# AO33/HiC_Genome_Assembler

Hardware: AMD Instinct MI355X
Metric: Part1+Part2 wall-clock (s) and bins/s on N x N contact map (higher is better)
Workload: dtype f64

## Files before the change

hic_genome_assembler_amd/csrc/api.hip:

```cpp
#include <hip/hip_runtime.h>

#include <algorithm>
#include <cmath>
#include <cstdarg>
#include <climits>
#include <cstdio>
#include <cstdlib>
#include <cstring>
#include <numeric>
#include <string>
#include <unordered_map>
#include <functional>
#include <chrono>
#include <vector>

#include "../../include/hicmi.h"
#include "hicmi_internal.h"
#include "hyper.h"

using namespace hicmi;

static thread_local std::string g_err;

static int fail(int code, const char* fmt, ...)
// ... 1150 lines not shown
    const uint16_t* src = c->dRank + row0 * c->ldr;
    HIPCHK(hipMemcpy2DAsync(out, sizeof(uint16_t) * (size_t)c->n, src, sizeof(uint16_t) * (size_t)c->ldr,
                            sizeof(uint16_t) * (size_t)c->n, (size_t)nrows, hipMemcpyDeviceToHost, c->stream));
    HIPCHK(sync_stream(c));
    if (!inverse) {
        std::vector<uint16_t> tmp((size_t)c->n);
        for (int64_t r = 0; r < nrows; r++) {
            uint16_t* row = out + r * c->n;
            for (int64_t col = 0; col < c->n; col++) {
                if (row[col] >= c->n) return fail(HICMI_ESTATE, "rank row %lld is not a permutation (a row of another shard?)", (long long)(row0 + r));
                tmp[row[col]] = (uint16_t)col;
            }
            memcpy(row, tmp.data(), sizeof(uint16_t) * (size_t)c->n);
        }
    }
    return HICMI_OK;
}

int hicmi_get_similarity_row(hicmi_ctx* c, int64_t row, double* out)
{
    if (!c || !out) return fail(HICMI_EINVAL, "bad arguments");
    if (!c->have_rank) return fail(HICMI_EINVAL, "hicmi_rank_matrix has not run");
    if (row < 0 || row >= c->n) return fail(HICMI_EINVAL, "row out of range");
    HIPCHK(hipSetDevice(c->device));
    int rc = ensure(c->d_tmp, c->tmp_cap, c->n);
    if (rc) return rc;
    launch_similarity_row(c->dC, c->ldc, c->d_order, c->d_np, c->d_seq, (int)c->n, (int)row, c->d_tmp, c->stream);
    HIPCHK(hipGetLastError());
    HIPCHK(hipMemcpyAsync(out, c->d_tmp, sizeof(double) * (size_t)c->n, hipMemcpyDeviceToHost, c->stream));
    HIPCHK(sync_stream(c));
    return HICMI_OK;
}

static int ensure_scan_buffers(hicmi_ctx* c)
{
    if (c->x_cap >= c->n && c->d_x && c->d_sig) return HICMI_OK;
    free_dev(c->d_x); free_dev(c->d_sig); c->d_x = nullptr; c->d_sig = nullptr; c->x_cap = 0;
    HIPCHK(hipMalloc((void**)&c->d_x, sizeof(int32_t) * (size_t)c->n));
    HIPCHK(hipMalloc((void**)&c->d_sig, (size_t)c->n));
    c->x_cap = c->n;
    return HICMI_OK;
}

static int finish_scan(hicmi_ctx* c, int64_t rows, int mode, int64_t L_fixed, int64_t M, double psig, int32_t* x_out,
                       uint8_t* sig_out, int64_t own_first)
{
    const bool direct = sig_out && !x_out;
    if (direct) { int rc = ensure_pin_down(c, (size_t)rows); if (rc) return rc; }
    {
        Timed t(c, F_HYPER_FLAGS, 5.0 * (double)rows);
        launch_hyper_flags(c->d_x, (int)rows, mode, (int)L_fixed, M, psig, direct ? reinterpret_cast<uint8_t*>(c->pin_down) : c->d_sig,
                           (int)own_first, (int)c->shard_stride, c->stream);
    }
    HIPCHK(hipGetLastError());
    if (direct) {
        HIPCHK(sync_stream(c));
        memcpy(sig_out, c->pin_down, (size_t)rows);
        return HICMI_OK;
    }
    if (x_out) { int rc = download(c, x_out, c->d_x, sizeof(int32_t) * (size_t)rows); if (rc) return rc; }
    if (sig_out) { int rc = download(c, sig_out, c->d_sig, (size_t)rows); if (rc) return rc; }
    if (!x_out && !sig_out) HIPCHK(sync_stream(c));
    return HICMI_OK;
}

int hicmi_cut_scan(hicmi_ctx* c, int64_t start, int64_t M, double psig, int32_t* x_out, uint8_t* sig_out)
{
    if (!c) return fail(HICMI_EINVAL, "NULL context");
    if (!c->have_rank) return fail(HICMI_EINVAL, "hicmi_rank_matrix has not run");
    const int64_t n = c->n;
    if (start < 0 || start >= n) return fail(HICMI_EINVAL, "start out of range");
    HIPCHK(hipSetDevice(c->device));
    int rc = ensure_scan_buffers(c);
    if (rc) return rc;
    const int64_t cnt = n - start;
    const int64_t st = c->shard_stride;
    const int64_t t0 = ((c->shard_first - start) % st + st) % st;
    if (c->cached_start != start) {
        HIPCHK(hipMemsetAsync(c->d_x, 0, sizeof(int32_t) * (size_t)(st > 1 ? cnt : 1), c->stream));
        const double m = (double)(cnt - 1);
        Timed t(c, F_CUT_COUNT, 2.0 * (m * (m + 3.0) / 2.0) / (double)st);
        const int64_t t1 = t0 >= 1 ? t0 : t0 + st;
        if (t1 < cnt)
            launch_cut_count(c->dRank, c->ldr, (int)(start + t1), (int)(cnt - t1), (int)start, 0, 0, c->d_x + t1, (int)st, c->stream);
        HIPCHK(hipGetLastError());
        c->cached_start = start;
    }
    return finish_scan(c, cnt, 0, 0, M, psig, x_out, sig_out, t0);
}

int hicmi_filter_scan(hicmi_ctx* c, int64_t start, int64_t cut, int64_t n_rows, int64_t M, double psig,
                      int32_t* x_out, uint8_t* sig_out)
{
    if (!c) return fail(HICMI_EINVAL, "NULL context");
    if (!c->have_rank) return fail(HICMI_EINVAL, "hicmi_rank_matrix has not run");
    const int64_t n = c->n;
    if (start < 0 || start >= n || cut < start || cut >= n || n_rows < 0 || start + n_rows > n)
        return fail(HICMI_EINVAL, "filter scan arguments out of range");
    HIPCHK(hipSetDevice(c->device));
    int rc = ensure_scan_buffers(c);
    if (rc) return rc;
    c->cached_start = -1;
    const int64_t st = c->shard_stride;
    const int64_t t0 = ((c->shard_first - start) % st + st) % st;
    if (st > 1) HIPCHK(hipMemsetAsync(c->d_x, 0, sizeof(int32_t) * (size_t)n_rows, c->stream));
    {
        Timed t(c, F_CUT_COUNT, 2.0 * (double)n_rows * (double)(cut - start + 1) / (double)st);
        if (t0 < n_rows)
            launch_cut_count(c->dRank, c->ldr, (int)(start + t0), (int)(n_rows - t0), (int)start, 1, (int)cut, c->d_x + t0, (int)st,
                             c->stream);
    }
    HIPCHK(hipGetLastError());
    return finish_scan(c, n_rows, 1, cut - start, M, psig, x_out, sig_out, t0);
}

double hicmi_hypergeom_sf(int64_t x, int64_t M, int64_t n, int64_t N) { return hypergeom_sf_ge(x, M, n, N); }
int hicmi_hypergeom_decide(int64_t x, int64_t M, int64_t n, int64_t N, double psig) { return hypergeom_decide(x, M, n, N, psig); }

static_assert(SCAN_MAX_SETS == HICMI_SCAN_MAX_SETS, "hicmi.h and the kernels disagree on the set cap");

struct ScanMulti {
    ScanState* st; int32_t *x, *cuts, *mlog, *alt, *seg, *seg_x; uint8_t *sig, *filt, *prev;
};

static int ensure_scan_multi(hicmi_ctx* c, int sets, ScanMulti& m)
{
    const size_t n = (size_t)c->n, S = (size_t)sets;
    const size_t head = (sizeof(ScanState) * SCAN_MAX_SETS + 255) & ~(size_t)255;
    const size_t bytes = head + S * n * (sizeof(int32_t) * 9 + 3) + 64;
    if (c->scan_multi_bytes < bytes || !c->d_scan_multi) {
        free_dev(c->d_scan_multi); c->d_scan_multi = nullptr; c->scan_multi_bytes = 0;
        HIPCHK(hipMalloc((void**)&c->d_scan_multi, bytes));
        c->scan_multi_bytes = bytes;
    }
    unsigned char* b = c->d_scan_multi;
    m.st = reinterpret_cast<ScanState*>(b);
    m.x = reinterpret_cast<int32_t*>(b + head);
    m.cuts = m.x + S * n; m.mlog = m.cuts + S * n; m.alt = m.mlog + 2 * S * n; m.seg = m.alt + S * n; m.seg_x = m.seg + 3 * S * n;
    m.sig = reinterpret_cast<uint8_t*>(m.seg_x + S * n); m.filt = m.sig + S * n; m.prev = m.filt + S * n;
    return HICMI_OK;
}

static int scan_share()
{
    const char* e = getenv("HICMI_SCAN_SHARE");
    return e && !strcmp(e, "0") ? 0 : 1;
}

static int run_scan_multi(hicmi_ctx* c, std::vector<ScanState>& h, const ScanMulti& m, const std::vector<int64_t>& max_scans,
                          const std::function<void(int)>& enqueue)
{
    const size_t S = h.size();
    int rc = upload(c, m.st, h.data(), sizeof(ScanState) * S);
    if (rc) return rc;
    const int pairs = 32;
    int64_t batches = 0;
    for (int64_t issued = 0; ; issued += pairs) {
        bool all_done = true;
        for (size_t k = 0; k < S; k++) {
            if (h[k].done) continue;
            all_done = false;
            if (issued > max_scans[k] + pairs)
                return fail(HICMI_ESTATE, "scan loop of set %d did not end after %lld scans", (int)k, (long long)issued);
        }
        if (all_done) break;
        {
            Timed t(c, F_CUT_COUNT, 0.0);
            enqueue(pairs);
        }
        HIPCHK(hipGetLastError());
        batches++;
        rc = download(c, h.data(), m.st, sizeof(ScanState) * S);
        if (rc) return rc;
    }
    int64_t scans = 0; double bytes = 0;
    for (const ScanState& r : h) { scans += r.scans; bytes += (double)r.bytes; }
    c->launches[F_CUT_COUNT] += scans - batches;
    c->launches[F_HYPER_FLAGS] += scans;
    c->bytes[F_CUT_COUNT] += bytes;
    return HICMI_OK;
}

static ScanState first_pass_record(int64_t n, int64_t min_size, int64_t stop_ind, double psig)
{
    ScanState r;
    memset(&r, 0, sizeof(r));
    r.mode = 0; r.start = 0; r.M = n; r.recount = 1; r.psig = psig;
    r.min_size = (int)std::min<int64_t>(min_size, n + 1); r.stop_ind = (int)std::min<int64_t>(stop_ind, INT32_MAX);
    return r;
}

static ScanState filter_record(int64_t n, int64_t n_in, int32_t first, double psig)
{
    ScanState r;
    memset(&r, 0, sizeof(r));
    r.mode = 1; r.start = 0; r.M = n; r.recount = 1; r.psig = psig;
    r.MD = (int)(n / 5);
    r.n_alt = (int)n_in; r.f_max_rounds = (int)std::min<int64_t>(10 * n_in, INT32_MAX);
    r.cut = first;
    r.n_rows = (int)std::min<int64_t>(n, (int64_t)r.MD + 1);
    r.done = n_in == 0;
    return r;
}

int hicmi_first_pass_cuts(hicmi_ctx* c, int64_t min_size, int64_t stop_ind, double psig, int32_t* cuts_out, int64_t cuts_cap,
                          int64_t* n_cuts_out, int32_t* m_log_out, int64_t log_cap, int64_t* n_log_out)
{
    return hicmi_first_pass_cuts_multi(c, 1, &min_size, &stop_ind, psig, cuts_out, cuts_cap, n_cuts_out, m_log_out, log_cap,
                                       n_log_out);
}

int hicmi_filter_cuts(hicmi_ctx* c, const int32_t* cuts_in, int64_t n_in, double psig, int32_t* cuts_out, int64_t cuts_cap,
                      int64_t* n_out, int64_t* warned_out)
{
    if (!c || !cuts_in || !cuts_out || !n_out || n_in < 1) return fail(HICMI_EINVAL, "bad arguments");
    const int64_t cand_off[2] = {0, n_in};
    int64_t warned = 0;
    const int rc = hicmi_filter_cuts_multi(c, 1, cand_off, cuts_in, &psig, cuts_out, cuts_cap, n_out, &warned);
    if (!rc && warned_out) *warned_out = warned;
    return rc;
}

int hicmi_first_pass_cuts_multi(hicmi_ctx* c, int64_t n_sets, const int64_t* min_size, const int64_t* stop_ind, double psig,
                                int32_t* cuts_out, int64_t cuts_cap, int64_t* n_cuts_out, int32_t* m_log_out, int64_t log_cap,
                                int64_t* n_log_out)
{
    if (!c || !min_size || !stop_ind || !cuts_out || !n_cuts_out || !n_log_out || (log_cap > 0 && !m_log_out))
        return fail(HICMI_EINVAL, "bad arguments");
    if (n_sets < 1 || n_sets > SCAN_MAX_SETS) return fail(HICMI_EINVAL, "n_sets must be in [1, %d]", SCAN_MAX_SETS);
    if (!c->have_rank) return fail(HICMI_EINVAL, "hicmi_rank_matrix has not run");
    if (c->shard_stride != 1) return fail(HICMI_EINVAL, "the device-driven scan loops need the whole rank matrix (no row shard)");
    for (int64_t k = 0; k < n_sets; k++)
        if (min_size[k] < 1) return fail(HICMI_EINVAL, "min_size must be >= 1 (set %lld)", (long long)k);
    const int64_t n = c->n;
    HIPCHK(hipSetDevice(c->device));
    ScanMulti m;
    int rc = ensure_scan_multi(c, (int)n_sets, m);
    if (rc) return rc;
    std::vector<ScanState> h((size_t)n_sets);
    for (int64_t k = 0; k < n_sets; k++) h[(size_t)k] = first_pass_record(n, min_size[k], stop_ind[k], psig);
    const int lcap = (int)n;
    const int share = scan_share();
    rc = run_scan_multi(c, h, m, std::vector<int64_t>((size_t)n_sets, 6 * n), [&](int pairs) {
        launch_first_pass_multi_pairs(c->dRank, c->ldr, (int)n, (int)n_sets, m.st, m.x, m.sig, psig, share, m.cuts, m.mlog,
                                      lcap, pairs, c->stream);
    });
    if (rc) return rc;
    for (int64_t k = 0; k < n_sets; k++) {
        const ScanState& r = h[(size_t)k];
        if (r.n_cuts > cuts_cap) return fail(HICMI_EINVAL, "%d cuts of set %lld do not fit cuts_cap", r.n_cuts, (long long)k);
        if (r.n_log > lcap || r.n_log > log_cap) return fail(HICMI_EINVAL, "%d M changes of set %lld do not fit the log", r.n_log, (long long)k);
    }
    for (int64_t k = 0; k < n_sets; k++) {
        const ScanState& r = h[(size_t)k];
        if (r.n_cuts) { rc = download(c, cuts_out + k * cuts_cap, m.cuts + k * n, sizeof(int32_t) * (size_t)r.n_cuts); if (rc) return rc; }
        if (r.n_log) { rc = download(c, m_log_out + 2 * k * log_cap, m.mlog + 2 * k * n, sizeof(int32_t) * 2 * (size_t)r.n_log); if (rc) return rc; }
        n_cuts_out[k] = r.n_cuts; n_log_out[k] = r.n_log;
    }
    return HICMI_OK;
}

int hicmi_filter_cuts_multi(hicmi_ctx* c, int64_t n_sets, const int64_t* cand_off, const int32_t* cuts_in, const double* psig,
                            int32_t* cuts_out, int64_t cuts_cap, int64_t* n_out, int64_t* warned_out)
{
    if (!c || !cand_off || !psig || !cuts_out || !n_out || !warned_out) return fail(HICMI_EINVAL, "bad arguments");
    if (n_sets < 1 || n_sets > SCAN_MAX_SETS) return fail(HICMI_EINVAL, "n_sets must be in [1, %d]", SCAN_MAX_SETS);
    if (!c->have_rank) return fail(HICMI_EINVAL, "hicmi_rank_matrix has not run");
    if (c->shard_stride != 1) return fail(HICMI_EINVAL, "the device-driven scan loops need the whole rank matrix (no row shard)");
    const int64_t n = c->n;
    if (cand_off[0] != 0) return fail(HICMI_EINVAL, "cand_off[0] must be 0");
    for (int64_t k = 0; k < n_sets; k++) {
        const int64_t a = cand_off[k], b = cand_off[k + 1];
        if (b < a || b - a > n) return fail(HICMI_EINVAL, "candidate list %lld: bad offsets", (long long)k);
        if (b > a && !cuts_in) return fail(HICMI_EINVAL, "bad arguments");
        for (int64_t i = a; i < b; i++)
            if (cuts_in[i] < 0 || cuts_in[i] >= n || (i > a && cuts_in[i] <= cuts_in[i - 1]))
                return fail(HICMI_EINVAL, "cuts must be ascending indices in [0, n) (set %lld)", (long long)k);
    }
    HIPCHK(hipSetDevice(c->device));
    ScanMulti m;
    int rc = ensure_scan_multi(c, (int)n_sets, m);
    if (rc) return rc;
    HIPCHK(hipMemsetAsync(m.filt, 0, 2 * (size_t)n_sets * (size_t)n, c->stream));
    std::vector<ScanState> h((size_t)n_sets);
    std::vector<int64_t> max_scans((size_t)n_sets);
    const int max_rows = (int)std::min<int64_t>(n, n / 5 + 1);
    for (int64_t k = 0; k < n_sets; k++) {
        const int64_t a = cand_off[k], n_in = cand_off[k + 1] - a;
        h[(size_t)k] = filter_record(n, n_in, n_in ? cuts_in[a] : 0, psig[k]);
        max_scans[(size_t)k] = std::min<int64_t>((int64_t)4000000, 20 * n_in * n_in * 10 + 1000);
        if (n_in) { rc = upload(c, m.alt + k * n, cuts_in + a, sizeof(int32_t) * (size_t)n_in); if (rc) return rc; }
    }
    const int share = scan_share();
    rc = run_scan_multi(c, h, m, max_scans, [&](int pairs) {
        launch_filter_multi_pairs(c->dRank, c->ldr, (int)n, max_rows, (int)n_sets, m.st, m.x, m.sig, psig[0], share, m.alt,
                                  m.filt, m.prev, m.seg, m.seg_x, pairs, c->stream);
    });
    if (rc) return rc;
    std::vector<uint8_t> kept((size_t)n_sets * (size_t)n);
    rc = download(c, kept.data(), m.filt, kept.size());
    if (rc) return rc;
    for (int64_t k = 0; k < n_sets; k++) {
        int64_t cnt = 0;
        const uint8_t* f = kept.data() + (size_t)k * (size_t)n;
        for (int64_t e = 0; e < n; e++)
            if (f[e]) {
                if (cnt >= cuts_cap) return fail(HICMI_EINVAL, "filtered cuts of set %lld do not fit cuts_cap", (long long)k);
                cuts_out[k * cuts_cap + cnt++] = (int32_t)e;
            }
        n_out[k] = cnt;
        warned_out[k] = h[(size_t)k].f_warned;
    }
    return HICMI_OK;
}

namespace {
void harmonic_table(std::vector<double>& H, int64_t n)
{
    H.assign((size_t)(n + 1), 0.0);
    for (int64_t k = 1; k <= n; k++) H[(size_t)k] = H[(size_t)k - 1] + 1.0 / (double)k;
}

int select_enqueue(hicmi_ctx* c, const int32_t* sel, int64_t n, const std::vector<double>* H_shared)
{
    if (!c || !sel || n < 1) return fail(HICMI_EINVAL, "bad arguments");
    if (!c->dC) return fail(HICMI_EINVAL, "no contact matrix set");
    for (int64_t i = 0; i < n; i++)
        if (sel[i] < 0 || sel[i] >= c->n) return fail(HICMI_EINVAL, "selection index out of range");
    HIPCHK(hipSetDevice(c->device));
// ... 2143 lines not shown
```

hic_genome_assembler_amd/csrc/hicmi_internal.h:

```cpp
#pragma once
#include <hip/hip_runtime.h>
#include <stdint.h>

#include <atomic>
#include <functional>

namespace hicmi {

inline void ensure_dynamic_lds(const void* func, std::atomic<int>& have, size_t bytes)
{
    if ((int)bytes > have.load(std::memory_order_relaxed)) {
        (void)hipFuncSetAttribute(func, hipFuncAttributeMaxDynamicSharedMemorySize, (int)bytes);
        have.store((int)bytes, std::memory_order_relaxed);
    }
}

static constexpr int SERIAL_BATCH = 16;

__device__ __forceinline__ double serial_sum_lds(const double* t, int from, int to, double acc)
{
    constexpr int B = SERIAL_BATCH;
    int i = from;
    if (i + B <= to) {
        double a[B];
// ... 88 lines not shown
    int dcap = 256;
    bool dcap_forced = false;
    bool compact = true;
    bool wgs_set = false; int wgs = 0;
    bool plain = false;
    bool gsize = false;
    bool w1 = true;
    int w1_s = 0;
    int w1_cols = 0;
    int w1_maxs = 0;
    int xcc = -1;
    int test_late = 0, test_diverge = 0, test_rollcall = 0;
};
NNChainOptions nnchain_options(int probed_xcc);
int nnchain_probe_xcc(hipStream_t s);
int launch_nnchain(double* W, double* W2, int64_t ldw, int n, int* chain, double* zraw, void* workspace, const NNChainOptions& o,
                   int fallback, hipStream_t s, const std::function<void()>& after_first_rowmin = nullptr);
void launch_selftest_division(unsigned long long seed, int blocks, int iters, unsigned long long* d_mismatches, hipStream_t s);
const int* nnchain_state_ptr(void* workspace);
const unsigned long long* nnchain_prof_ptr(void* workspace);
void launch_cut_count(const uint16_t* rank, int64_t ldr, int row0, int nrows, int lo, int mode, int cparam,
                      int32_t* x_out, int row_step, hipStream_t s);
void launch_hyper_flags(const int32_t* x, int nrows, int mode, int L_fixed, int64_t M, double psig, uint8_t* sig,
                        int own_first, int own_step, hipStream_t s);

struct ScanState {
    int done;
    int mode;
    int start, cut, n_rows, recount;
    long long M;
    double psig;
    int min_size, stop_ind, loop_count, n_cuts, n_log, scans;
    int MD, n_alt, alt_off, f_i, f_keep_from, f_noise, f_round, f_max_rounds, f_warned;
    int pad;
    unsigned long long bytes;
};
static constexpr int SCAN_MAX_SETS = 64;
void launch_first_pass_multi_pairs(const uint16_t* rank, int64_t ldr, int n, int n_sets, ScanState* st, int32_t* x, uint8_t* sig,
                                   double psig0, int share, int32_t* cuts, int32_t* mlog, int log_cap, int pairs, hipStream_t s);
void launch_filter_multi_pairs(const uint16_t* rank, int64_t ldr, int n, int max_rows, int n_sets, ScanState* st, int32_t* x,
                               uint8_t* sig, double psig0, int share, int32_t* alt, uint8_t* filt, uint8_t* prev,
                               int32_t* seg, int32_t* seg_x, int pairs, hipStream_t s);

#if defined(__HIPCC__)
template <int M>
__device__ __forceinline__ uint32_t xor_lane(uint32_t v, int lane)
{
    if constexpr (M == 1) return (uint32_t)__builtin_amdgcn_mov_dpp((int)v, 0xB1, 0xf, 0xf, true);
    else if constexpr (M == 2) return (uint32_t)__builtin_amdgcn_mov_dpp((int)v, 0x4E, 0xf, 0xf, true);
    else if constexpr (M == 4) {
        const int t = __builtin_amdgcn_mov_dpp((int)v, 0x141, 0xf, 0xf, true);
        return (uint32_t)__builtin_amdgcn_mov_dpp(t, 0x1B, 0xf, 0xf, true);
    } else if constexpr (M == 8) {
        const int t = __builtin_amdgcn_mov_dpp((int)v, 0x140, 0xf, 0xf, true);
        return (uint32_t)__builtin_amdgcn_mov_dpp(t, 0x141, 0xf, 0xf, true);
    } else if constexpr (M == 16) {
        const auto r = __builtin_amdgcn_permlane16_swap(v, v, false, false);
        return (lane & 16) ? r[0] : r[1];
    } else {
        static_assert(M == 32, "xor_lane: M must be 1, 2, 4, 8, 16 or 32");
        const auto r = __builtin_amdgcn_permlane32_swap(v, v, false, false);
        return (lane & 32) ? r[0] : r[1];
    }
}
#endif

int  sort_padded_size(int n);
int  sort_workgroups(int n);
size_t sort_scratch_bytes(int n);
struct SortExtras {
    const int32_t* row_list = nullptr; int n_list = 0;
    uint8_t* tie_flag = nullptr; unsigned* tie_count = nullptr; unsigned tie_limit = 0;
    uint16_t* tie_bits = nullptr; int64_t ld_bits = 0;
    int max_workgroups = 0;
    int avoid_xcc = -1; unsigned* row_counter = nullptr;
// ... 240 lines not shown
```

hic_genome_assembler_amd/csrc/k_part1_scan.hip:

```cpp
#include "hicmi_internal.h"
#include "hyper.h"

namespace hicmi {

__device__ __forceinline__ int row_count_partial(const uint16_t* __restrict__ r, int lo, int end, int thr, int tid)
{
    int cnt = 0;
    int body0 = (lo + 7) & ~7;
    if (body0 > end) body0 = end;
    const int body1 = body0 + ((end - body0) & ~7);
    for (int j = lo + tid; j < body0; j += 256) cnt += (int)r[j] < thr;
    for (int j = body0 + tid * 8; j < body1; j += 256 * 8) {
        uint4 q = *reinterpret_cast<const uint4*>(r + j);
        cnt += (int)(q.x & 0xffffu) < thr; cnt += (int)(q.x >> 16) < thr;
        cnt += (int)(q.y & 0xffffu) < thr; cnt += (int)(q.y >> 16) < thr;
        cnt += (int)(q.z & 0xffffu) < thr; cnt += (int)(q.z >> 16) < thr;
        cnt += (int)(q.w & 0xffffu) < thr; cnt += (int)(q.w >> 16) < thr;
    }
    for (int j = body1 + tid; j < end; j += 256) cnt += (int)r[j] < thr;
    return cnt;
}

__device__ __forceinline__ uint8_t row_flag(int mode, int total, long long M, int t, int thr, double psig)
{
// ... 2 lines not shown
}

__global__ __launch_bounds__(256) void k_cut_rows(const uint16_t* __restrict__ rank, int64_t ldr, int n,
                                                  const ScanState* __restrict__ st, int32_t* __restrict__ x,
                                                  uint8_t* __restrict__ sig, double psig)
{
    __shared__ int s_part[4];
    if (st->done) return;
    const int mode = st->mode, lo = st->start, t = blockIdx.x;
    const int rows = mode == 0 ? n - lo : st->n_rows;
    if (t >= rows) return;
    const int tid = threadIdx.x;
    if (mode == 0 && t == 0) { if (tid == 0) sig[0] = 0; return; }
    const int i = lo + t;
    const int hi = mode == 0 ? i : st->cut;
    const int thr = hi - lo;
    int total;
    if (st->recount) {
        int cnt = row_count_partial(rank + (int64_t)i * ldr, lo, hi + 1, thr, tid);
#pragma unroll
        for (int off = 32; off >= 1; off >>= 1) cnt += __shfl_xor(cnt, off, 64);
        if ((tid & 63) == 0) s_part[tid >> 6] = cnt;
        __syncthreads();
        if (tid != 0) return;
        total = s_part[0] + s_part[1] + s_part[2] + s_part[3];
        x[t] = total;
    } else {
        if (tid != 0) return;
        total = x[t];
    }
    sig[t] = row_flag(mode, total, st->M, t, thr, psig);
}

__device__ __forceinline__ void first_pass_decide(int n, ScanState* __restrict__ st, const uint8_t* __restrict__ sig,
                                                  int32_t* __restrict__ cuts, int32_t* __restrict__ mlog, int log_cap)
{
    __shared__ int s_sum[16];
    __shared__ int s_first;
    __shared__ int s_go;
    if (st->done) return;
    const int tid = threadIdx.x;
    const int start = st->start, cnt = n - start, h = st->min_size;
    int part = 0;
    for (int e = tid; e < cnt; e += 1024) part += sig[e];
#pragma unroll
    for (int off = 32; off >= 1; off >>= 1) part += __shfl_xor(part, off, 64);
    if ((tid & 63) == 0) s_sum[tid >> 6] = part;
    if (tid == 0) s_first = 0x7fffffff;
    __syncthreads();
    if (tid == 0) {
        int total = 0;
        for (int w = 0; w < 16; w++) total += s_sum[w];
        int go = 1;
        st->scans++;
        if (st->recount) { const unsigned long long m = (unsigned long long)(cnt - 1); st->bytes += m * (m + 3); }
        st->loop_count++;
        if ((double)total / (double)cnt >= .9) {
            const int64_t morg = st->M;
            st->M = morg - start;
            if (st->n_log < log_cap) { mlog[2 * st->n_log] = (int32_t)morg; mlog[2 * st->n_log + 1] = (int32_t)st->M; }
            st->n_log++;
            if (st->loop_count < 5) { go = 0; st->recount = 0; }
        }
        s_go = go;
    }
    __syncthreads();
    if (!s_go) return;
    const int full = cnt - 2 * h + 1;
    if (h < cnt) {
        for (int p = tid; p < full; p += 1024) {
            bool ok = true;
            for (int k = 0; k < h && ok; k++) ok = sig[p + k] == 1 && sig[p + h + k] == 0;
            if (ok) { atomicMin(&s_first, p); break; }
        }
    }
    __syncthreads();
    if (tid != 0) return;
    if (s_first == 0x7fffffff) { st->done = 1; return; }
    const int ind = start + s_first + h;
    cuts[st->n_cuts++] = ind;
    if (ind >= st->stop_ind || (n - ind) <= h) { st->done = 1; return; }
    st->start = ind; st->M = n - ind; st->loop_count = 0; st->recount = 1;
}

__device__ __forceinline__ void filter_begin_round(ScanState* st, int n)
{
    st->M = n - st->start;
    st->f_i = 0;
    st->f_keep_from = 0;
}

__device__ __forceinline__ void filter_set_scan(ScanState* st, const int32_t* alt, int n)
{
    st->cut = alt[st->alt_off + st->f_i];
    const int rest = n - st->start;
    st->n_rows = rest < st->MD + 1 ? rest : st->MD + 1;
    st->recount = 1;
}

static constexpr int FD_CAP = 2048;

__device__ __forceinline__ void filter_decide(int n, ScanState* __restrict__ st, const uint8_t* __restrict__ sig,
                                              int32_t* __restrict__ alt, uint8_t* __restrict__ filt,
                                              uint8_t* __restrict__ prev, int32_t* __restrict__ seg_g,
                                              int32_t* __restrict__ seg_x_g, double psig)
{
    __shared__ int s_alt[FD_CAP], s_seg[3 * FD_CAP], s_seg_x[FD_CAP];
    __shared__ int s_nseg, s_last, s_phase, s_diff, s_wave[16];
    if (st->done) return;
    const int tid = threadIdx.x;
    const int start = st->start, c = st->cut, n_rows = st->n_rows, n_alt = st->n_alt - st->alt_off;
    const bool in_lds = n_alt <= FD_CAP;
    int* a = in_lds ? s_alt : alt + st->alt_off;
    int* seg = in_lds ? s_seg : seg_g;
    int* seg_x = in_lds ? s_seg_x : seg_x_g;
    if (in_lds)
        for (int k = tid; k < n_alt; k += 1024) s_alt[k] = alt[st->alt_off + k];
    __syncthreads();
    if (tid == 0) {
        int ns = 0, fc_prev = start;
        for (int k = 0; k < n_alt; k++) {
            const int ai = a[k];
            if (ai == fc_prev) continue;
            const int lo = fc_prev, hi = ai;
            fc_prev = ai;
            if (hi <= lo) break;
            seg[3 * ns] = lo; seg[3 * ns + 1] = hi; seg[3 * ns + 2] = k;
            seg_x[ns] = 0;
            ns++;
        }
        s_nseg = ns; s_last = -1;
        st->scans++;
        st->bytes += 2ull * (unsigned long long)n_rows * (unsigned long long)(c - start + 1);
    }
    __syncthreads();
    const int ns = s_nseg;
    for (int e = tid; e < n_rows; e += 1024) {
        if (!sig[e]) continue;
        const int row = start + e;
        int lo_k = 0, hi_k = ns;
        while (lo_k < hi_k) {
            const int mid = (lo_k + hi_k) >> 1;
            if (seg[3 * mid + 1] > row) hi_k = mid; else lo_k = mid + 1;
        }
        if (lo_k < ns && seg[3 * lo_k] <= row) atomicAdd(&seg_x[lo_k], 1);
    }
    __syncthreads();
    const int64_t M = st->M;
    const int local = c - start;
    for (int k = tid; k < ns; k += 1024) {
        const double p = hypergeom_sf_ge((int64_t)seg_x[k], M, (int64_t)local, (int64_t)(seg[3 * k + 1] - seg[3 * k]));
        if (p < psig) atomicMax(&s_last, k);
    }
    __syncthreads();
    if (tid == 0) {
        int phase = 0;
        if (s_last >= 0) {
            st->f_keep_from = seg[3 * s_last + 2];
            st->start = seg[3 * s_last + 1];
            filt[st->start] = 1;
            st->f_noise = 1;
            phase = 1;
        } else {
            filt[c] = 1;
            st->f_keep_from = st->f_i;
            st->f_i++;
            if (st->f_i >= n_alt) phase = 1;
        }
        if (phase == 1) {
            st->f_round++;
            if (st->f_noise == 0) phase = 2;
            else {
                st->alt_off += st->f_keep_from;
                st->f_noise = 0;
                if (st->f_round >= st->f_max_rounds) { st->f_warned++; phase = 2; }
                else if (st->alt_off >= st->n_alt) phase = 2;
                else filter_begin_round(st, n);
            }
        }
        s_phase = phase;
        s_diff = 0;
    }
    __syncthreads();
    if (s_phase != 2) {
        if (tid == 0) filter_set_scan(st, alt, n);
        return;
    }
    __threadfence_block();
    const int chunk = (n + 1023) / 1024;
    const int e0 = tid * chunk, e1 = e0 + chunk < n ? e0 + chunk : n;
    int mine = 0, diff = 0;
    for (int e = e0; e < e1; e++) { const int f = filt[e]; mine += f; diff |= f != prev[e]; }
    if (diff) s_diff = 1;
    int incl = mine;
#pragma unroll
    for (int d = 1; d < 64; d <<= 1) { const int o = __shfl_up(incl, d, 64); if ((tid & 63) >= d) incl += o; }
    if ((tid & 63) == 63) s_wave[tid >> 6] = incl;
    __syncthreads();
    if (!s_diff) { if (tid == 0) st->done = 1; return; }
    int base = incl - mine, total = 0;
// ... 49 lines not shown
    }
    __syncthreads();
    const int items = s_pre[n_sets];
    for (int w = blockIdx.x; w < items; w += gridDim.x) {
        int k = 0;
        while (s_pre[k + 1] <= w) k++;
        const int t = w - s_pre[k];
        const int mode = s_key[k][1], lo = s_key[k][2];
        if (mode == 0 && t == 0) {
            if (tid < n_sets && s_lead[tid] == k) sig[(size_t)tid * n] = 0;
            continue;
        }
        const int i = lo + t;
        const int hi = mode == 0 ? i : st[k].cut;
        const int thr = hi - lo;
        if (s_key[k][3] >= 0) {
            int cnt = row_count_partial(rank + (int64_t)i * ldr, lo, hi + 1, thr, tid);
#pragma unroll
            for (int off = 32; off >= 1; off >>= 1) cnt += __shfl_xor(cnt, off, 64);
            if ((tid & 63) == 0) s_part[tid >> 6] = cnt;
            __syncthreads();
            const int total = s_part[0] + s_part[1] + s_part[2] + s_part[3];
            if (tid < n_sets && s_lead[tid] == k) {
                x[(size_t)tid * n + t] = total;
                sig[(size_t)tid * n + t] = row_flag(mode, total, st[tid].M, t, thr, st[tid].psig);
            }
            __syncthreads();
        } else if (tid == 0) {
            sig[(size_t)k * n + t] = row_flag(mode, x[(size_t)k * n + t], st[k].M, t, thr, st[k].psig);
        }
    }
}

__global__ __launch_bounds__(1024) void k_first_pass_decide_multi(int n, ScanState* __restrict__ st, const uint8_t* __restrict__ sig,
                                                                  int32_t* __restrict__ cuts, int32_t* __restrict__ mlog, int log_cap)
{
    const size_t k = blockIdx.x;
    first_pass_decide(n, st + k, sig + k * n, cuts + k * n, mlog + k * 2 * n, log_cap);
}

__global__ __launch_bounds__(1024) void k_filter_decide_multi(int n, ScanState* __restrict__ st, const uint8_t* __restrict__ sig,
                                                              int32_t* __restrict__ alt, uint8_t* __restrict__ filt,
                                                              uint8_t* __restrict__ prev, int32_t* __restrict__ seg_g,
                                                              int32_t* __restrict__ seg_x_g)
{
    const size_t k = blockIdx.x;
    filter_decide(n, st + k, sig + k * n, alt + k * n, filt + k * n, prev + k * n, seg_g + k * 3 * n, seg_x_g + k * n,
                  st[k].psig);
}

static void launch_cut_rows(const uint16_t* rank, int64_t ldr, int n, int rows, int n_sets, const ScanState* st, int32_t* x,
                            uint8_t* sig, double psig0, int share, hipStream_t s)
{
    if (n_sets == 1) hipLaunchKernelGGL(k_cut_rows, dim3(rows), dim3(256), 0, s, rank, ldr, n, st, x, sig, psig0);
    else hipLaunchKernelGGL(k_cut_rows_multi, dim3(rows), dim3(256), 0, s, rank, ldr, n, n_sets, st, x, sig, share);
}

void launch_first_pass_multi_pairs(const uint16_t* rank, int64_t ldr, int n, int n_sets, ScanState* st, int32_t* x, uint8_t* sig,
                                   double psig0, int share, int32_t* cuts, int32_t* mlog, int log_cap, int pairs, hipStream_t s)
{
    for (int k = 0; k < pairs; k++) {
        launch_cut_rows(rank, ldr, n, n, n_sets, st, x, sig, psig0, share, s);
        hipLaunchKernelGGL(k_first_pass_decide_multi, dim3(n_sets), dim3(1024), 0, s, n, st, sig, cuts, mlog, log_cap);
    }
}

void launch_filter_multi_pairs(const uint16_t* rank, int64_t ldr, int n, int max_rows, int n_sets, ScanState* st, int32_t* x,
                               uint8_t* sig, double psig0, int share, int32_t* alt, uint8_t* filt, uint8_t* prev,
                               int32_t* seg, int32_t* seg_x, int pairs, hipStream_t s)
{
    for (int k = 0; k < pairs; k++) {
        launch_cut_rows(rank, ldr, n, max_rows, n_sets, st, x, sig, psig0, share, s);
        hipLaunchKernelGGL(k_filter_decide_multi, dim3(n_sets), dim3(1024), 0, s, n, st, sig, alt, filt, prev, seg, seg_x);
    }
}

}
```

Before: 125,800.

## Add wave-per-row cut scans, multi-cut lookahead filter, and adaptive batch sizing

Adds wave-per-row counting kernels that read rank rows as 128-bit vectors and reduce with wave shuffles. It also adds a lookahead filter that scores up to four candidate cuts per scan and packs two cuts' segment counts into one atomic word. The host now sizes each scan batch from an estimate of the scans left, and environment switches choose between the plain and wave forms. The aim is fewer serial scan iterations and launches and better bandwidth per row, at the cost of speculative work for cuts that end up discarded and more complex state.

```diff
diff --git a/hic_genome_assembler_amd/csrc/api.hip b/hic_genome_assembler_amd/csrc/api.hip
--- a/hic_genome_assembler_amd/csrc/api.hip
+++ b/hic_genome_assembler_amd/csrc/api.hip
@@ -1206,6 +1206,8 @@
     return HICMI_OK;
 }
 
+static int scan_form();
+
 static int ensure_scan_buffers(hicmi_ctx* c)
 {
     if (c->x_cap >= c->n && c->d_x && c->d_sig) return HICMI_OK;
@@ -1255,7 +1257,9 @@
         const double m = (double)(cnt - 1);
         Timed t(c, F_CUT_COUNT, 2.0 * (m * (m + 3.0) / 2.0) / (double)st);
         const int64_t t1 = t0 >= 1 ? t0 : t0 + st;
-        if (t1 < cnt)
+        if (t1 < cnt && st == 1 && scan_form() != SCAN_PLAIN)
+            launch_cut_count_wave(c->dRank, c->ldr, (int)(start + t1), (int)(cnt - t1), (int)start, 0, 0, c->d_x + t1, c->stream);
+        else if (t1 < cnt)
             launch_cut_count(c->dRank, c->ldr, (int)(start + t1), (int)(cnt - t1), (int)start, 0, 0, c->d_x + t1, (int)st, c->stream);
         HIPCHK(hipGetLastError());
         c->cached_start = start;
@@ -1280,7 +1284,10 @@
     if (st > 1) HIPCHK(hipMemsetAsync(c->d_x, 0, sizeof(int32_t) * (size_t)n_rows, c->stream));
     {
         Timed t(c, F_CUT_COUNT, 2.0 * (double)n_rows * (double)(cut - start + 1) / (double)st);
-        if (t0 < n_rows)
+        if (t0 < n_rows && st == 1 && scan_form() != SCAN_PLAIN)
+            launch_cut_count_wave(c->dRank, c->ldr, (int)(start + t0), (int)(n_rows - t0), (int)start, 1, (int)cut, c->d_x + t0,
+                                  c->stream);
+        else if (t0 < n_rows)
             launch_cut_count(c->dRank, c->ldr, (int)(start + t0), (int)(n_rows - t0), (int)start, 1, (int)cut, c->d_x + t0, (int)st,
                              c->stream);
     }
@@ -1321,23 +1328,56 @@
     return e && !strcmp(e, "0") ? 0 : 1;
 }
 
+static int scan_form()
+{
+    const char* e = getenv("HICMI_SCAN_PLAIN");
+    if (e && !strcmp(e, "1")) return SCAN_PLAIN;
+    e = getenv("HICMI_SCAN_WAVE");
+    if (e && !strcmp(e, "1")) return SCAN_WAVE;
+    if (e && !strcmp(e, "64")) return SCAN_WAVE64;
+    return SCAN_AUTO;
+}
+
+static int scan_look_max(int64_t n_sets)
+{
+    const char* e = getenv("HICMI_SCAN_LOOK");
+    if (!e || !*e) return n_sets == 1 ? 2 : 1;
+    const int v = atoi(e);
+    return v < 1 ? 1 : v > 4 ? 4 : v;
+}
+
+static int scans_ahead(const ScanState& r, int64_t n)
+{
+    if (r.done) return 0;
+    if (r.mode == 0) {
+        if (r.start <= 0 || r.scans <= 0) return 32;
+        const int64_t end = std::min<int64_t>(r.stop_ind, n - r.min_size);
+        const int64_t left = std::max<int64_t>(end - r.start, 0);
+        return (int)std::min<int64_t>(32, left * r.scans / r.start + 2);
+    }
+    return (int)std::min<int64_t>(32, (int64_t)(r.n_alt - r.alt_off - r.f_i) + 2);
+}
+
 static int run_scan_multi(hicmi_ctx* c, std::vector<ScanState>& h, const ScanMulti& m, const std::vector<int64_t>& max_scans,
-                          const std::function<void(int)>& enqueue)
+                          bool fixed_batches, const std::function<void(int)>& enqueue)
 {
     const size_t S = h.size();
     int rc = upload(c, m.st, h.data(), sizeof(ScanState) * S);
     if (rc) return rc;
-    const int pairs = 32;
+    int pairs = 32;
     int64_t batches = 0;
     for (int64_t issued = 0; ; issued += pairs) {
         bool all_done = true;
+        int ahead = 0;
         for (size_t k = 0; k < S; k++) {
             if (h[k].done) continue;
             all_done = false;
-            if (issued > max_scans[k] + pairs)
+            if (issued > max_scans[k] + 32)
                 return fail(HICMI_ESTATE, "scan loop of set %d did not end after %lld scans", (int)k, (long long)issued);
+            ahead = std::max(ahead, scans_ahead(h[k], c->n));
         }
         if (all_done) break;
+        pairs = fixed_batches || batches == 0 ? 32 : std::min(32, std::max(8, ahead));
         {
             Timed t(c, F_CUT_COUNT, 0.0);
             enqueue(pairs);
@@ -1364,8 +1404,9 @@
     return r;
 }
 
-static ScanState filter_record(int64_t n, int64_t n_in, int32_t first, double psig)
-{
+static ScanState filter_record(int64_t n, int64_t n_in, const int32_t* cand, double psig, int look_max)
+{
+    const int32_t first = n_in ? cand[0] : 0;
     ScanState r;
     memset(&r, 0, sizeof(r));
     r.mode = 1; r.start = 0; r.M = n; r.recount = 1; r.psig = psig;
@@ -1373,6 +1414,13 @@
     r.n_alt = (int)n_in; r.f_max_rounds = (int)std::min<int64_t>(10 * n_in, INT32_MAX);
     r.cut = first;
     r.n_rows = (int)std::min<int64_t>(n, (int64_t)r.MD + 1);
+    r.look_max = look_max;
+    int64_t B = std::min<int64_t>(look_max, n_in);
+    if (n_in > 2048) B = std::min<int64_t>(B, 2);
+    B = std::max<int64_t>(1, std::min<int64_t>(B, n / ((int64_t)r.MD + 1)));
+    r.look = (int)B;
+    r.look_cut[0] = first;
+    for (int64_t b = 1; b < B; b++) r.look_cut[b] = cand[b];
     r.done = n_in == 0;
     return r;
 }
@@ -1414,10 +1462,10 @@
     std::vector<ScanState> h((size_t)n_sets);
     for (int64_t k = 0; k < n_sets; k++) h[(size_t)k] = first_pass_record(n, min_size[k], stop_ind[k], psig);
     const int lcap = (int)n;
-    const int share = scan_share();
-    rc = run_scan_multi(c, h, m, std::vector<int64_t>((size_t)n_sets, 6 * n), [&](int pairs) {
-        launch_first_pass_multi_pairs(c->dRank, c->ldr, (int)n, (int)n_sets, m.st, m.x, m.sig, psig, share, m.cuts, m.mlog,
-                                      lcap, pairs, c->stream);
+    const int share = scan_share(), form = scan_form();
+    rc = run_scan_multi(c, h, m, std::vector<int64_t>((size_t)n_sets, 6 * n), form == SCAN_PLAIN || form == SCAN_AUTO, [&](int pairs) {
+        launch_first_pass_multi_pairs(c->dRank, c->ldr, (int)n, (int)n_sets, m.st, m.x, m.sig, psig, share, form, m.cuts,
+                                      m.mlog, lcap, pairs, c->stream);
     });
     if (rc) return rc;
     for (int64_t k = 0; k < n_sets; k++) {
@@ -1456,19 +1504,20 @@
     int rc = ensure_scan_multi(c, (int)n_sets, m);
     if (rc) return rc;
     HIPCHK(hipMemsetAsync(m.filt, 0, 2 * (size_t)n_sets * (size_t)n, c->stream));
+    const int share = scan_share(), form = scan_form();
+    const int look_max = form == SCAN_PLAIN ? 1 : scan_look_max(n_sets);
     std::vector<ScanState> h((size_t)n_sets);
     std::vector<int64_t> max_scans((size_t)n_sets);
     const int max_rows = (int)std::min<int64_t>(n, n / 5 + 1);
     for (int64_t k = 0; k < n_sets; k++) {
         const int64_t a = cand_off[k], n_in = cand_off[k + 1] - a;
-        h[(size_t)k] = filter_record(n, n_in, n_in ? cuts_in[a] : 0, psig[k]);
+        h[(size_t)k] = filter_record(n, n_in, cuts_in + a, psig[k], look_max);
         max_scans[(size_t)k] = std::min<int64_t>((int64_t)4000000, 20 * n_in * n_in * 10 + 1000);
         if (n_in) { rc = upload(c, m.alt + k * n, cuts_in + a, sizeof(int32_t) * (size_t)n_in); if (rc) return rc; }
     }
-    const int share = scan_share();
-    rc = run_scan_multi(c, h, m, max_scans, [&](int pairs) {
-        launch_filter_multi_pairs(c->dRank, c->ldr, (int)n, max_rows, (int)n_sets, m.st, m.x, m.sig, psig[0], share, m.alt,
-                                  m.filt, m.prev, m.seg, m.seg_x, pairs, c->stream);
+    rc = run_scan_multi(c, h, m, max_scans, form == SCAN_PLAIN, [&](int pairs) {
+        launch_filter_multi_pairs(c->dRank, c->ldr, (int)n, max_rows, (int)n_sets, m.st, m.x, m.sig, psig[0], share, form,
+                                  look_max, m.alt, m.filt, m.prev, m.seg, m.seg_x, pairs, c->stream);
     });
     if (rc) return rc;
     std::vector<uint8_t> kept((size_t)n_sets * (size_t)n);
diff --git a/hic_genome_assembler_amd/csrc/hicmi_internal.h b/hic_genome_assembler_amd/csrc/hicmi_internal.h
--- a/hic_genome_assembler_amd/csrc/hicmi_internal.h
+++ b/hic_genome_assembler_amd/csrc/hicmi_internal.h
@@ -144,15 +144,20 @@
     double psig;
     int min_size, stop_ind, loop_count, n_cuts, n_log, scans;
     int MD, n_alt, alt_off, f_i, f_keep_from, f_noise, f_round, f_max_rounds, f_warned;
+    int look, look_max, look_cut[4];
     int pad;
     unsigned long long bytes;
 };
 static constexpr int SCAN_MAX_SETS = 64;
+enum { SCAN_PLAIN = 0, SCAN_WAVE = 1, SCAN_WAVE64 = 2, SCAN_AUTO = 3 };
 void launch_first_pass_multi_pairs(const uint16_t* rank, int64_t ldr, int n, int n_sets, ScanState* st, int32_t* x, uint8_t* sig,
-                                   double psig0, int share, int32_t* cuts, int32_t* mlog, int log_cap, int pairs, hipStream_t s);
+                                   double psig0, int share, int form, int32_t* cuts, int32_t* mlog, int log_cap, int pairs,
+                                   hipStream_t s);
 void launch_filter_multi_pairs(const uint16_t* rank, int64_t ldr, int n, int max_rows, int n_sets, ScanState* st, int32_t* x,
-                               uint8_t* sig, double psig0, int share, int32_t* alt, uint8_t* filt, uint8_t* prev,
-                               int32_t* seg, int32_t* seg_x, int pairs, hipStream_t s);
+                               uint8_t* sig, double psig0, int share, int form, int look, int32_t* alt, uint8_t* filt,
+                               uint8_t* prev, int32_t* seg, int32_t* seg_x, int pairs, hipStream_t s);
+void launch_cut_count_wave(const uint16_t* rank, int64_t ldr, int row0, int nrows, int lo, int mode, int cparam, int32_t* x_out,
+                           hipStream_t s);
 
 #if defined(__HIPCC__)
 template <int M>
diff --git a/hic_genome_assembler_amd/csrc/k_part1_scan.hip b/hic_genome_assembler_amd/csrc/k_part1_scan.hip
--- a/hic_genome_assembler_amd/csrc/k_part1_scan.hip
+++ b/hic_genome_assembler_amd/csrc/k_part1_scan.hip
@@ -58,6 +58,90 @@
     sig[t] = row_flag(mode, total, st->M, t, thr, psig);
 }
 
+__device__ __forceinline__ int row_count_wave(const uint16_t* __restrict__ r, int lo, int end, int thr, int lane)
+{
+    int cnt = 0;
+    int body0 = (lo + 7) & ~7;
+    if (body0 > end) body0 = end;
+    const int body1 = body0 + ((end - body0) & ~7);
+    for (int j = lo + lane; j < body0; j += 64) cnt += (int)r[j] < thr;
+#pragma unroll 4
+    for (int j = body0 + lane * 8; j < body1; j += 64 * 8) {
+        uint4 q = *reinterpret_cast<const uint4*>(r + j);
+        cnt += (int)(q.x & 0xffffu) < thr; cnt += (int)(q.x >> 16) < thr;
+        cnt += (int)(q.y & 0xffffu) < thr; cnt += (int)(q.y >> 16) < thr;
+        cnt += (int)(q.z & 0xffffu) < thr; cnt += (int)(q.z >> 16) < thr;
+        cnt += (int)(q.w & 0xffffu) < thr; cnt += (int)(q.w >> 16) < thr;
+    }
+    for (int j = body1 + lane; j < end; j += 64) cnt += (int)r[j] < thr;
+#pragma unroll
+    for (int off = 32; off >= 1; off >>= 1) cnt += __shfl_xor(cnt, off, 64);
+    return cnt;
+}
+
+template <bool DECIDE64>
+__global__ __launch_bounds__(DECIDE64 ? 1024 : 256) void k_cut_rows_wave(const uint16_t* __restrict__ rank, int64_t ldr, int n,
+                                                       const ScanState* __restrict__ st, int32_t* __restrict__ x,
+                                                       uint8_t* __restrict__ sig, double psig)
+{
+    constexpr int ROWS = DECIDE64 ? 64 : 4;
+    constexpr int PER_WAVE = DECIDE64 ? 4 : 1;
+    __shared__ int s_cnt[64];
+    if (st->done) return;
+    const int mode = st->mode, lo = st->start;
+    const int n_rows = mode == 0 ? n - lo : st->n_rows;
+    const int rows = mode == 0 ? n_rows : n_rows * st->look;
+    const long long M = st->M;
+    const int tid = threadIdx.x, lane = tid & 63, wave = tid >> 6;
+    if (!st->recount) {
+        const int t = blockIdx.x * (int)blockDim.x + tid;
+        if (t >= rows) return;
+        if (mode == 0 && t == 0) { sig[0] = 0; return; }
+        sig[t] = row_flag(mode, x[t], M, t, mode == 0 ? t : st->look_cut[t / n_rows] - lo, psig);
+        return;
+    }
+    const int G = (rows + ROWS - 1) / ROWS, b = blockIdx.x;
+    if (b >= G) return;
+#pragma unroll 1
+    for (int k = 0; k < PER_WAVE; k++) {
+        const int j = DECIDE64 ? k * 16 + wave : wave;
+        const int t = DECIDE64 ? j * G + b : b * ROWS + j;
+        if (t >= rows) break;
+        if (mode == 0 && t == 0) { if (lane == 0) sig[0] = 0; continue; }
+        const int i = mode == 0 ? lo + t : lo + t % n_rows;
+        const int hi = mode == 0 ? i : st->look_cut[t / n_rows];
+        const int total = row_count_wave(rank + (int64_t)i * ldr, lo, hi + 1, hi - lo, lane);
+        if (lane == 0) {
+            x[t] = total;
+            if (DECIDE64) s_cnt[j] = total;
+            else sig[t] = row_flag(mode, total, M, t, hi - lo, psig);
+        }
+    }
+    if (!DECIDE64) return;
+    __syncthreads();
+    const int t = tid * G + b;
+    if (tid >= 64 || t >= rows || (mode == 0 && t == 0)) return;
+    sig[t] = row_flag(mode, s_cnt[tid], M, t, mode == 0 ? t : st->look_cut[t / n_rows] - lo, psig);
+}
+
+__global__ __launch_bounds__(256) void k_cut_count_wave(const uint16_t* __restrict__ rank, int64_t ldr, int row0, int nrows,
+                                                        int lo, int mode, int cparam, int32_t* __restrict__ x_out)
+{
+    const int t = blockIdx.x * 4 + (threadIdx.x >> 6);
+    if (t >= nrows) return;
+    const int i = row0 + t;
+    const int hi = mode == 0 ? i : cparam;
+    const int total = row_count_wave(rank + (int64_t)i * ldr, lo, hi + 1, hi - lo, threadIdx.x & 63);
+    if ((threadIdx.x & 63) == 0) x_out[t] = total;
+}
+
+void launch_cut_count_wave(const uint16_t* rank, int64_t ldr, int row0, int nrows, int lo, int mode, int cparam, int32_t* x_out,
+                           hipStream_t s)
+{
+    if (nrows <= 0) return;
+    hipLaunchKernelGGL(k_cut_count_wave, dim3((nrows + 3) / 4), dim3(256), 0, s, rank, ldr, row0, nrows, lo, mode, cparam, x_out);
+}
+
 __device__ __forceinline__ void first_pass_decide(int n, ScanState* __restrict__ st, const uint8_t* __restrict__ sig,
                                                   int32_t* __restrict__ cuts, int32_t* __restrict__ mlog, int log_cap)
 {
@@ -116,26 +200,33 @@
     st->f_keep_from = 0;
 }
 
+static constexpr int FD_CAP = 2048;
+
 __device__ __forceinline__ void filter_set_scan(ScanState* st, const int32_t* alt, int n)
 {
-    st->cut = alt[st->alt_off + st->f_i];
     const int rest = n - st->start;
     st->n_rows = rest < st->MD + 1 ? rest : st->MD + 1;
     st->recount = 1;
-}
-
-static constexpr int FD_CAP = 2048;
+    const int left = st->n_alt - st->alt_off - st->f_i;
+    int B = st->look_max < left ? st->look_max : left;
+    if (st->n_alt - st->alt_off > FD_CAP && B > 2) B = 2;
+    if (B > n / (st->MD + 1)) B = n / (st->MD + 1);
+    if (B < 1) B = 1;
+    for (int b = 0; b < B; b++) st->look_cut[b] = alt[st->alt_off + st->f_i + b];
+    st->look = B;
+    st->cut = st->look_cut[0];
+}
 
 __device__ __forceinline__ void filter_decide(int n, ScanState* __restrict__ st, const uint8_t* __restrict__ sig,
                                               int32_t* __restrict__ alt, uint8_t* __restrict__ filt,
                                               uint8_t* __restrict__ prev, int32_t* __restrict__ seg_g,
                                               int32_t* __restrict__ seg_x_g, double psig)
 {
-    __shared__ int s_alt[FD_CAP], s_seg[3 * FD_CAP], s_seg_x[FD_CAP];
-    __shared__ int s_nseg, s_last, s_phase, s_diff, s_wave[16];
+    __shared__ int s_alt[FD_CAP], s_seg[3 * FD_CAP], s_seg_x[2 * FD_CAP];
+    __shared__ int s_nseg, s_last[4], s_phase, s_diff, s_wave[16];
     if (st->done) return;
     const int tid = threadIdx.x;
-    const int start = st->start, c = st->cut, n_rows = st->n_rows, n_alt = st->n_alt - st->alt_off;
+    const int start = st->start, n_rows = st->n_rows, n_alt = st->n_alt - st->alt_off, B = st->look;
     const bool in_lds = n_alt <= FD_CAP;
     int* a = in_lds ? s_alt : alt + st->alt_off;
     int* seg = in_lds ? s_seg : seg_g;
@@ -152,46 +243,53 @@
             fc_prev = ai;
             if (hi <= lo) break;
             seg[3 * ns] = lo; seg[3 * ns + 1] = hi; seg[3 * ns + 2] = k;
-            seg_x[ns] = 0;
             ns++;
         }
-        s_nseg = ns; s_last = -1;
-        st->scans++;
-        st->bytes += 2ull * (unsigned long long)n_rows * (unsigned long long)(c - start + 1);
+        s_nseg = ns;
+        s_last[0] = s_last[1] = s_last[2] = s_last[3] = -1;
     }
     __syncthreads();
     const int ns = s_nseg;
-    for (int e = tid; e < n_rows; e += 1024) {
-        if (!sig[e]) continue;
-        const int row = start + e;
+    for (int k = tid; k < ((B + 1) >> 1) * ns; k += 1024) seg_x[k] = 0;
+    __syncthreads();
+    for (int t = tid; t < B * n_rows; t += 1024) {
+        if (!sig[t]) continue;
+        const int b = t / n_rows, row = start + t % n_rows;
         int lo_k = 0, hi_k = ns;
         while (lo_k < hi_k) {
             const int mid = (lo_k + hi_k) >> 1;
             if (seg[3 * mid + 1] > row) hi_k = mid; else lo_k = mid + 1;
         }
-        if (lo_k < ns && seg[3 * lo_k] <= row) atomicAdd(&seg_x[lo_k], 1);
+        if (lo_k < ns && seg[3 * lo_k] <= row) atomicAdd(&seg_x[(b >> 1) * ns + lo_k], 1 << (16 * (b & 1)));
     }
     __syncthreads();
     const int64_t M = st->M;
-    const int local = c - start;
-    for (int k = tid; k < ns; k += 1024) {
-        const double p = hypergeom_sf_ge((int64_t)seg_x[k], M, (int64_t)local, (int64_t)(seg[3 * k + 1] - seg[3 * k]));
-        if (p < psig) atomicMax(&s_last, k);
+    for (int t = tid; t < B * ns; t += 1024) {
+        const int b = t / ns, k = t % ns;
+        const int local = st->look_cut[b] - start;
+        const int xk = (seg_x[(b >> 1) * ns + k] >> (16 * (b & 1))) & 0xffff;
+        const double p = hypergeom_sf_ge((int64_t)xk, M, (int64_t)local, (int64_t)(seg[3 * k + 1] - seg[3 * k]));
+        if (p < psig) atomicMax(&s_last[b], k);
     }
     __syncthreads();
     if (tid == 0) {
         int phase = 0;
-        if (s_last >= 0) {
-            st->f_keep_from = seg[3 * s_last + 2];
-            st->start = seg[3 * s_last + 1];
-            filt[st->start] = 1;
-            st->f_noise = 1;
-            phase = 1;
-        } else {
-            filt[c] = 1;
-            st->f_keep_from = st->f_i;
-            st->f_i++;
-            if (st->f_i >= n_alt) phase = 1;
+        for (int b = 0; b < B && phase == 0; b++) {
+            const int c = st->look_cut[b];
+            st->scans++;
+            st->bytes += 2ull * (unsigned long long)n_rows * (unsigned long long)(c - start + 1);
+            if (s_last[b] >= 0) {
+                st->f_keep_from = seg[3 * s_last[b] + 2];
+                st->start = seg[3 * s_last[b] + 1];
+                filt[st->start] = 1;
+                st->f_noise = 1;
+                phase = 1;
+            } else {
+                filt[c] = 1;
+                st->f_keep_from = st->f_i;
+                st->f_i++;
+                if (st->f_i >= n_alt) phase = 1;
+            }
         }
         if (phase == 1) {
             st->f_round++;
@@ -307,6 +405,83 @@
     }
 }
 
+__global__ __launch_bounds__(256) void k_cut_rows_multi_wave(const uint16_t* __restrict__ rank, int64_t ldr, int n, int n_sets,
+                                                             const ScanState* __restrict__ st, int32_t* __restrict__ x,
+                                                             uint8_t* __restrict__ sig, int share)
+{
+    static_assert(SCAN_MAX_SETS <= 64, "a wave's lanes are the sets an item serves");
+    __shared__ int s_pre[SCAN_MAX_SETS + 1];
+    __shared__ int s_lead[SCAN_MAX_SETS];
+    __shared__ int s_key[SCAN_MAX_SETS][4];
+    __shared__ int s_cut[SCAN_MAX_SETS][4];
+    __shared__ int s_rows[SCAN_MAX_SETS][2];
+    const int tid = threadIdx.x, lane = tid & 63, wave = tid >> 6;
+    if (tid < SCAN_MAX_SETS) {
+        int live = 0, mode = 0, start = 0, recount = 0, rows = 0, n_rows = 1;
+        int cut[4] = {-1, -1, -1, -1};
+        if (tid < n_sets && !st[tid].done) {
+            live = 1; mode = st[tid].mode; start = st[tid].start; recount = st[tid].recount != 0;
+            n_rows = mode == 0 ? n - start : st[tid].n_rows;
+            rows = mode == 0 ? n_rows : n_rows * st[tid].look;
+            if (mode == 1)
+                for (int b = 0; b < 4; b++) if (b < st[tid].look) cut[b] = st[tid].look_cut[b];
+        }
+        s_key[tid][0] = live; s_key[tid][1] = mode; s_key[tid][2] = start; s_key[tid][3] = recount;
+        for (int b = 0; b < 4; b++) s_cut[tid][b] = cut[b];
+        s_lead[tid] = live && recount ? tid : -1;
+        s_rows[tid][0] = rows; s_rows[tid][1] = n_rows > 0 ? n_rows : 1;
+    }
+    __syncthreads();
+    if (tid < SCAN_MAX_SETS) {
+        int rows = s_key[tid][0] && s_key[tid][3] ? s_rows[tid][0] : 0;
+        if (share && rows) {
+            for (int j = 0; j < tid; j++)
+                if (s_key[j][0] && s_key[j][3] && s_key[j][1] == s_key[tid][1] && s_key[j][2] == s_key[tid][2] &&
+                    s_cut[j][0] == s_cut[tid][0] && s_cut[j][1] == s_cut[tid][1] && s_cut[j][2] == s_cut[tid][2] &&
+                    s_cut[j][3] == s_cut[tid][3]) {
+                    s_lead[tid] = j; rows = 0; break;
+                }
+        }
+        int incl = rows;
+#pragma unroll
+        for (int d = 1; d < 64; d <<= 1) { const int o = __shfl_up(incl, d, 64); if (tid >= d) incl += o; }
+        s_pre[tid + 1] = incl;
+        if (tid == 0) s_pre[0] = 0;
+    }
+    __syncthreads();
+    const int items = s_pre[n_sets];
+    for (int w = blockIdx.x * 4 + wave; w < items; w += gridDim.x * 4) {
+        int k = 0;
+        while (s_pre[k + 1] <= w) k++;
+        const int t = w - s_pre[k];
+        const int mode = s_key[k][1], lo = s_key[k][2];
+        const bool mine = lane < n_sets && s_lead[lane] == k;
+        if (mode == 0 && t == 0) {
+            if (mine) sig[(size_t)lane * n] = 0;
+            continue;
+        }
+        const int i = mode == 0 ? lo + t : lo + t % s_rows[k][1];
+        const int hi = mode == 0 ? i : s_cut[k][t / s_rows[k][1]];
+        const int thr = hi - lo;
+        const int total = row_count_wave(rank + (int64_t)i * ldr, lo, hi + 1, thr, lane);
+        if (mine) {
+            x[(size_t)lane * n + t] = total;
+            sig[(size_t)lane * n + t] = row_flag(mode, total, st[lane].M, t, thr, st[lane].psig);
+        }
+    }
+    for (int k = 0; k < n_sets; k++) {
+        if (!s_key[k][0] || s_key[k][3]) continue;
+        const int mode = s_key[k][1], rows = s_rows[k][0];
+        const long long M = st[k].M;
+        const double psig = st[k].psig;
+        for (int t = blockIdx.x * 256 + tid; t < rows; t += gridDim.x * 256) {
+            if (mode == 0 && t == 0) { sig[(size_t)k * n] = 0; continue; }
+            const int thr = mode == 0 ? t : s_cut[k][t / s_rows[k][1]] - s_key[k][2];
+            sig[(size_t)k * n + t] = row_flag(mode, x[(size_t)k * n + t], M, t, thr, psig);
+        }
+    }
+}
+
 __global__ __launch_bounds__(1024) void k_first_pass_decide_multi(int n, ScanState* __restrict__ st, const uint8_t* __restrict__ sig,
                                                                   int32_t* __restrict__ cuts, int32_t* __restrict__ mlog, int log_cap)
 {
@@ -325,27 +500,41 @@
 }
 
 static void launch_cut_rows(const uint16_t* rank, int64_t ldr, int n, int rows, int n_sets, const ScanState* st, int32_t* x,
-                            uint8_t* sig, double psig0, int share, hipStream_t s)
-{
-    if (n_sets == 1) hipLaunchKernelGGL(k_cut_rows, dim3(rows), dim3(256), 0, s, rank, ldr, n, st, x, sig, psig0);
-    else hipLaunchKernelGGL(k_cut_rows_multi, dim3(rows), dim3(256), 0, s, rank, ldr, n, n_sets, st, x, sig, share);
+                            uint8_t* sig, double psig0, int share, int form, int look, bool filter, hipStream_t s)
+{
+    if (form == SCAN_AUTO) form = n_sets == 1 ? (filter ? SCAN_WAVE64 : SCAN_PLAIN) : (look > 1 ? SCAN_WAVE : SCAN_PLAIN);
+    if (form == SCAN_PLAIN) {
+        if (n_sets == 1) hipLaunchKernelGGL(k_cut_rows, dim3(rows), dim3(256), 0, s, rank, ldr, n, st, x, sig, psig0);
+        else hipLaunchKernelGGL(k_cut_rows_multi, dim3(rows), dim3(256), 0, s, rank, ldr, n, n_sets, st, x, sig, share);
+    } else if (n_sets == 1) {
+        rows *= look;
+        if (form == SCAN_WAVE64)
+            hipLaunchKernelGGL(k_cut_rows_wave<true>, dim3((rows + 63) / 64), dim3(1024), 0, s, rank, ldr, n, st, x, sig, psig0);
+        else
+            hipLaunchKernelGGL(k_cut_rows_wave<false>, dim3((rows + 3) / 4), dim3(256), 0, s, rank, ldr, n, st, x, sig, psig0);
+    } else {
+        const int64_t want = ((int64_t)rows * look * n_sets + 3) / 4;
+        const int grid = (int)(want < 4096 ? want : 4096);
+        hipLaunchKernelGGL(k_cut_rows_multi_wave, dim3(grid), dim3(256), 0, s, rank, ldr, n, n_sets, st, x, sig, share);
+    }
 }
 
 void launch_first_pass_multi_pairs(const uint16_t* rank, int64_t ldr, int n, int n_sets, ScanState* st, int32_t* x, uint8_t* sig,
-                                   double psig0, int share, int32_t* cuts, int32_t* mlog, int log_cap, int pairs, hipStream_t s)
+                                   double psig0, int share, int form, int32_t* cuts, int32_t* mlog, int log_cap, int pairs,
+                                   hipStream_t s)
 {
     for (int k = 0; k < pairs; k++) {
-        launch_cut_rows(rank, ldr, n, n, n_sets, st, x, sig, psig0, share, s);
+        launch_cut_rows(rank, ldr, n, n, n_sets, st, x, sig, psig0, share, form, 1, false, s);
         hipLaunchKernelGGL(k_first_pass_decide_multi, dim3(n_sets), dim3(1024), 0, s, n, st, sig, cuts, mlog, log_cap);
     }
 }
 
 void launch_filter_multi_pairs(const uint16_t* rank, int64_t ldr, int n, int max_rows, int n_sets, ScanState* st, int32_t* x,
-                               uint8_t* sig, double psig0, int share, int32_t* alt, uint8_t* filt, uint8_t* prev,
-                               int32_t* seg, int32_t* seg_x, int pairs, hipStream_t s)
+                               uint8_t* sig, double psig0, int share, int form, int look, int32_t* alt, uint8_t* filt,
+                               uint8_t* prev, int32_t* seg, int32_t* seg_x, int pairs, hipStream_t s)
 {
     for (int k = 0; k < pairs; k++) {
-        launch_cut_rows(rank, ldr, n, max_rows, n_sets, st, x, sig, psig0, share, s);
+        launch_cut_rows(rank, ldr, n, max_rows, n_sets, st, x, sig, psig0, share, form, look, true, s);
         hipLaunchKernelGGL(k_filter_decide_multi, dim3(n_sets), dim3(1024), 0, s, n, st, sig, alt, filt, prev, seg, seg_x);
     }
 }
```

Result: slower. 122,800 (-2.5%).
